# guanjq/targetdiff

Measured on AMD Instinct MI355X. Metric: ligands/sec (1000-step sampling, 100 samples/pocket) at 1/2/4/8 MI355X, higher is better.
Workload: dtype f32

## Files before the change

targetdiff_amd/csrc/node.hip:

```cpp

#include <type_traits>
#include "td_device.h"
#include "td_internal.h"

constexpr int NP_CHUNK_STEPS = 16;
constexpr int NP_CHUNK_F4 = NP_CHUNK_STEPS * 64;
constexpr int NP_CHUNKS = TD_KSTEPS / NP_CHUNK_STEPS;
constexpr int NP_TSTRIDE = 36;
constexpr size_t NP_LDS_BYTES = (size_t)(2 * NP_CHUNK_F4 * 4 + 4 * 32 * NP_TSTRIDE) * sizeof(float);

__device__ __forceinline__ void gemm128_lds(const float4 (&a)[16], const float4 *__restrict__ B,
                                            const float4 *__restrict__ next, float4 *__restrict__ bufs, int &cur,
                                            int tid, int lane, floatx16 (&acc)[4]) {
#pragma unroll
    for (int ch = 0; ch < NP_CHUNKS; ++ch) {
        const float4 *src = ch + 1 < NP_CHUNKS ? B + (size_t)(ch + 1) * NP_CHUNK_F4 : next;
        if (src) {
            float4 *dst = bufs + (cur ^ 1) * NP_CHUNK_F4 + (tid & ~63);
            const int nthr = blockDim.x;
            for (int u = 0; u < NP_CHUNK_F4; u += nthr) td_glds16(src + u + tid, dst + u);
        }
        const float4 *bl = bufs + cur * NP_CHUNK_F4 + lane;
#pragma unroll
        for (int s = 0; s < NP_CHUNK_STEPS; ++s) {
// ... 100 lines not shown
        int seen = 0;
        unsigned sel = 0;
        for (int b = 0; b < 5; ++b)
            if ((mat_mask >> b) & 1u) {
                if (seen == unit) sel = 1u << b;
                ++seen;
            }
        mat_mask = sel;
    }
    constexpr size_t MAT_F4 = (size_t)TD_KSTEPS * 64;
    const float4 *Bp = reinterpret_cast<const float4 *>(st.projB);
    const float4 *seq[6];
    int mats[6], nseq = 0;
    for (int mat = 0; mat < 5; ++mat)
        if ((mat_mask >> mat) & 1u) { seq[nseq] = Bp + (size_t)mat * MAT_F4; mats[nseq++] = mat; }
    if ((mat_mask >> 4) & 1u) { seq[nseq] = reinterpret_cast<const float4 *>(st.q3B); mats[nseq++] = 5; }
    for (int u = tid; u < NP_CHUNK_F4; u += blockDim.x) bufs[u] = seq[0][u];
    __syncthreads();
    int cur = 0;
    floatx16 acc[4];
    for (int si = 0; si < nseq; ++si) {
        const int mat = mats[si];
        const float *bias = mat < 5 ? st.projBias + mat * TD_H : st.q3Bias;
#pragma unroll
        for (int t = 0; t < 4; ++t) {
            const float bv = bias[32 * t + c];
#pragma unroll
            for (int r = 0; r < 16; ++r) acc[t][r] = bv;
        }
        const float4 *next = si + 1 < nseq ? seq[si + 1] : nullptr;
        gemm128_lds(a, seq[si], next, bufs, cur, tid, lane, acc);
        if (mat < 4) {
#pragma unroll
            for (int r = 0; r < 16; ++r) {
                const int orow = out_row(r);
                if (orow >= 0) {
#pragma unroll
                    for (int t = 0; t < 4; ++t) P[(size_t)orow * (4 * TD_H) + mat * TD_H + 32 * t + c] = acc[t][r];
                }
            }
        } else if (mat == 4) {
            float gam[4], bet[4];
#pragma unroll
            for (int t = 0; t < 4; ++t) {
                gam[t] = st.qGamma[32 * t + c];
                bet[t] = st.qBeta[32 * t + c];
            }
#pragma unroll
            for (int r = 0; r < 16; ++r) {
                const float s1 = (acc[0][r] + acc[1][r]) + (acc[2][r] + acc[3][r]);
                const float mean = td_sum32(s1) * (1.0f / TD_H);
                const float d0 = acc[0][r] - mean, d1 = acc[1][r] - mean, d2 = acc[2][r] - mean, d3 = acc[3][r] - mean;
                const float var = td_sum32((d0 * d0 + d1 * d1) + (d2 * d2 + d3 * d3)) * (1.0f / TD_H);
                const float rstd = __frsqrt_rn(var + 1e-5f);
                acc[0][r] = fmaxf(d0 * rstd * gam[0] + bet[0], 0.f);
                acc[1][r] = fmaxf(d1 * rstd * gam[1] + bet[1], 0.f);
                acc[2][r] = fmaxf(d2 * rstd * gam[2] + bet[2], 0.f);
                acc[3][r] = fmaxf(d3 * rstd * gam[3] + bet[3], 0.f);
            }
#pragma unroll
            for (int t = 0; t < 4; ++t) {
#pragma unroll
                for (int r = 0; r < 16; ++r) tb[td_erow(r, hi) * NP_TSTRIDE + c] = acc[t][r];
#pragma unroll
                for (int mm = 0; mm < 4; ++mm)
                    a[4 * t + mm] = *reinterpret_cast<const float4 *>(tb + c * NP_TSTRIDE + 8 * mm + 4 * hi);
            }
        } else {
#pragma unroll
            for (int r = 0; r < 16; ++r) {
                const int orow = out_row(r);
                if (orow >= 0) {
#pragma unroll
                    for (int t = 0; t < 4; ++t) q[(size_t)orow * TD_H + 32 * t + c] = acc[t][r];
                }
            }
        }
    }
}

__device__ __forceinline__ void td_glds16_asm_s(const uint4 *gsrc_base, uint32_t lane_bytes, uint32_t lds_wave_base) {
    asm volatile("s_mov_b32 m0, %2\n\ts_nop 0\n\tglobal_load_lds_dwordx4 %0, %1" : : "v"(lane_bytes), "s"(gsrc_base), "s"(lds_wave_base) : "memory", "m0");
}
template <bool ASYNC, bool BPIPE>
__global__ __launch_bounds__(256, 2) void node_proj_split_kernel(NpArgs args, const float *__restrict__ h) {
    int bx = blockIdx.x, si = 0;
    while (si + 1 < args.nseg && bx >= args.seg[si].blocks) { bx -= args.seg[si].blocks; ++si; }
    const NpSeg &sg = args.seg[si];
    const TdNodeStage st = sg.st;
    const int32_t *__restrict__ rows = sg.rows;
    float *__restrict__ P = sg.P, *__restrict__ q = sg.q;
    unsigned mat_mask = sg.mask;
    int64_t N = sg.N;
    int unit = -1;
    if (sg.units > 1) {
        unit = bx % sg.units;
        bx /= sg.units;
    }
    if (sg.count_ptr) {
        N = *sg.count_ptr;
        if ((int64_t)bx * (blockDim.x >> 1) >= N) return;
    }
    extern __shared__ __attribute__((aligned(16))) float lds[];
    uint4 *bufs = reinterpret_cast<uint4 *>(lds);
    const int tid = threadIdx.x, lane = tid & 63, wave = tid >> 6;
    float *tb = lds + 2 * NPS_CHUNK_U4 * 4 + wave * 32 * NP_TSTRIDE;
    const int c = lane & 31, hi = lane >> 5;
    const int64_t row0 = ((int64_t)bx * (blockDim.x >> 6) + wave) * 32;
    if (unit >= 0) {
        int seen = 0;
        unsigned sel = 0;
        for (int b = 0; b < 5; ++b)
            if ((mat_mask >> b) & 1u) {
                if (seen == unit) sel = 1u << b;
                ++seen;
            }
        mat_mask = sel;
    }
    const unsigned seq_mask = (mat_mask & 0x1fu) | (((mat_mask >> 4) & 1u) << 5);
    if (!seq_mask) return;
    constexpr size_t MAT_U4 = (size_t)NPS_CHUNKS * NPS_CHUNK_U4;
    const uint4 *Bp = reinterpret_cast<const uint4 *>(st.projB3), *Bq3 = reinterpret_cast<const uint4 *>(st.q3B3);
    auto mat_after = [&](int m) -> int {
        const unsigned rest = seq_mask & ~((2u << m) - 1u);
        return rest ? __builtin_ctz(rest) : -1;
    };
    auto mat_ptr = [&](int m) -> const uint4 * { return m < 5 ? Bp + (size_t)m * MAT_U4 : Bq3; };
    int mat = __builtin_ctz(seq_mask);
    float *sbias = lds + 2 * NPS_CHUNK_U4 * 4 + 4 * 32 * NP_TSTRIDE;
    {
        const uint4 *first = mat_ptr(mat);
        for (int u = tid; u < NPS_CHUNK_U4; u += blockDim.x) bufs[u] = first[u];
        for (int u = tid; u < NPS_BIAS_FLOATS; u += blockDim.x) sbias[u] = u < 5 * TD_H ? st.projBias[u] : st.q3Bias[u - 5 * TD_H];
    }
    uint4 ap[3][8];
    int orow4[4];
    {
        const int64_t aslot = row0 + c;
        const int64_t arow = aslot < N ? (rows ? (int64_t)rows[aslot] : aslot) : -1;
#pragma unroll
        for (int k = 0; k < 4; ++k) orow4[k] = __shfl((int)arow, (lane >> 3) + 8 * k);
        float4 a[16];
#pragma unroll
        for (int m = 0; m < 16; ++m)
            a[m] = (arow >= 0) ? *reinterpret_cast<const float4 *>(h + arow * TD_H + 8 * m + 4 * hi) : make_float4(0.f, 0.f, 0.f, 0.f);
        td_split_tile(a, ap);
    }
    __syncthreads();
    int cur = 0;
    const int64_t row0s = ((int64_t)bx * (blockDim.x >> 6) + __builtin_amdgcn_readfirstlane(wave)) * 32;
    const bool direct = !rows && row0s + 32 <= N;
    floatx16 keep[2];
    for (; mat >= 0; mat = mat_after(mat)) {
        const float *bias = sbias + mat * TD_H;
        const uint4 *B = mat_ptr(mat);
        const int mat_next = mat_after(mat);
#pragma unroll
        for (int half = 0; half < 2; ++half) {
            floatx16 acc[2];
#pragma unroll
            for (int t = 0; t < 2; ++t) {
                const float bv = bias[64 * half + 32 * t + c];
#pragma unroll
                for (int r = 0; r < 16; ++r) acc[t][r] = bv;
            }
#pragma unroll
            for (int kc = 0; kc < 2; ++kc) {
                const int chunk = 2 * half + kc;
                const uint4 *src = chunk + 1 < NPS_CHUNKS ? B + (size_t)(chunk + 1) * NPS_CHUNK_U4
                                                            : (mat_next >= 0 ? mat_ptr(mat_next) : nullptr);
                if constexpr (ASYNC) {
                    if (src) {
                        const uint32_t lbase = __builtin_amdgcn_readfirstlane(
                            (uint32_t)(uintptr_t)(__attribute__((address_space(3))) void *)(bufs + (cur ^ 1) * NPS_CHUNK_U4 + (tid & ~63)));
#pragma unroll
                        for (int u = 0; u < NPS_CHUNK_U4 / 256; ++u) {
                            td_glds16_asm_s(src + u * 256, (uint32_t)tid * 16u, lbase + u * 256 * 16);
                        }
                    }
                } else if (src) {
                    uint4 *dst = bufs + (cur ^ 1) * NPS_CHUNK_U4 + (tid & ~63);
                    for (int u = 0; u < NPS_CHUNK_U4; u += 256)
                        td_glds16(reinterpret_cast<const float4 *>(src + u + tid), reinterpret_cast<float4 *>(dst + u));
                }
                const uint4 *bl = bufs + cur * NPS_CHUNK_U4 + lane;
                uint4 b[2][3][2];
                auto load_b = [&](int ss, uint4 (&bb)[3][2]) {
#pragma unroll
                    for (int p = 0; p < 3; ++p)
#pragma unroll
                        for (int t = 0; t < 2; ++t) bb[p][t] = bl[((ss * 3 + p) * 2 + t) * 64];
                };
                if constexpr (BPIPE) load_b(0, b[0]);
#pragma unroll
                for (int ss = 0; ss < 4; ++ss) {
                    const int s = 4 * kc + ss;
                    uint4 (&bc)[3][2] = b[BPIPE ? (ss & 1) : 0];
                    if constexpr (BPIPE) {
                        if (ss + 1 < 4) load_b(ss + 1, b[(ss + 1) & 1]);
                        __builtin_amdgcn_sched_barrier(0);
                    } else
                        load_b(ss, bc);
#pragma unroll
                    for (int t = 0; t < 2; ++t) acc[t] = td_mfma_bf16(ap[1][s], bc[1][t], acc[t]);
#pragma unroll
                    for (int t = 0; t < 2; ++t) acc[t] = td_mfma_bf16(ap[2][s], bc[0][t], acc[t]);
#pragma unroll
                    for (int t = 0; t < 2; ++t) acc[t] = td_mfma_bf16(ap[0][s], bc[2][t], acc[t]);
#pragma unroll
                    for (int t = 0; t < 2; ++t) acc[t] = td_mfma_bf16(ap[1][s], bc[0][t], acc[t]);
#pragma unroll
                    for (int t = 0; t < 2; ++t) acc[t] = td_mfma_bf16(ap[0][s], bc[1][t], acc[t]);
#pragma unroll
                    for (int t = 0; t < 2; ++t) acc[t] = td_mfma_bf16(ap[0][s], bc[0][t], acc[t]);
                    if constexpr (BPIPE) __builtin_amdgcn_sched_barrier(0);
                }
                if constexpr (ASYNC) asm volatile("s_waitcnt vmcnt(0)" : : : "memory");
                __syncthreads();
                cur ^= 1;
            }
            if (mat != 4) {
                float *out = mat < 4 ? P + mat * TD_H + 64 * half : q + 64 * half;
                const size_t ld = mat < 4 ? (size_t)(4 * TD_H) : (size_t)TD_H;
                if (direct) {
                    auto store_tiles = [&](float *base, auto ldc) {
                        constexpr int LD = (int)decltype(ldc)::value;
                        const __amdgpu_buffer_rsrc_t rs = __builtin_amdgcn_make_buffer_rsrc(base + (size_t)row0s * LD, 0, 32 * LD * 4, 0x00020000);
                        const int voff = ((4 * hi) * LD + c) * 4;
#pragma unroll
                        for (int t = 0; t < 2; ++t)
#pragma unroll
                            for (int r = 0; r < 16; ++r)
                                __builtin_amdgcn_raw_buffer_store_b32(__float_as_uint(acc[t][r]), rs, voff, (td_erow(r, 0) * LD + 32 * t) * 4, 0);
                    };
                    if (mat < 4) store_tiles(out, std::integral_constant<int, 4 * TD_H>());
                    else store_tiles(out, std::integral_constant<int, TD_H>());
                } else
#pragma unroll
                for (int t = 0; t < 2; ++t) {
#pragma unroll
                    for (int r = 0; r < 16; ++r) tb[td_erow(r, hi) * NP_TSTRIDE + c] = acc[t][r];
#pragma unroll
                    for (int k = 0; k < 4; ++k) {
                        const float4 v = *reinterpret_cast<const float4 *>(tb + ((lane >> 3) + 8 * k) * NP_TSTRIDE + 4 * (lane & 7));
                        if (orow4[k] >= 0) *reinterpret_cast<float4 *>(out + (size_t)orow4[k] * ld + 32 * t + 4 * (lane & 7)) = v;
                    }
                }
            } else if (half == 0) {
                keep[0] = acc[0];
                keep[1] = acc[1];
            } else {
                float gam[4], bet[4];
#pragma unroll
                for (int t = 0; t < 4; ++t) {
                    gam[t] = st.qGamma[32 * t + c];
                    bet[t] = st.qBeta[32 * t + c];
                }
#pragma unroll
                for (int r = 0; r < 16; ++r) {
                    const float s1 = (keep[0][r] + keep[1][r]) + (acc[0][r] + acc[1][r]);
                    const float mean = td_sum32(s1) * (1.0f / TD_H);
                    const float d0 = keep[0][r] - mean, d1 = keep[1][r] - mean, d2 = acc[0][r] - mean, d3 = acc[1][r] - mean;
                    const float var = td_sum32((d0 * d0 + d1 * d1) + (d2 * d2 + d3 * d3)) * (1.0f / TD_H);
                    const float rstd = __frsqrt_rn(var + 1e-5f);
                    keep[0][r] = fmaxf(d0 * rstd * gam[0] + bet[0], 0.f);
                    keep[1][r] = fmaxf(d1 * rstd * gam[1] + bet[1], 0.f);
                    acc[0][r] = fmaxf(d2 * rstd * gam[2] + bet[2], 0.f);
                    acc[1][r] = fmaxf(d3 * rstd * gam[3] + bet[3], 0.f);
                }
                float4 a[16];
#pragma unroll
                for (int t = 0; t < 4; ++t) {
#pragma unroll
                    for (int r = 0; r < 16; ++r)
                        tb[td_erow(r, hi) * NP_TSTRIDE + c] = t == 0 ? keep[0][r] : t == 1 ? keep[1][r] : t == 2 ? acc[0][r] : acc[1][r];
#pragma unroll
                    for (int mm = 0; mm < 4; ++mm)
                        a[4 * t + mm] = *reinterpret_cast<const float4 *>(tb + c * NP_TSTRIDE + 8 * mm + 4 * hi);
                }
                td_split_tile(a, ap);
            }
        }
    }
}

static int np_fill(NpSeg &g, const TdNodeStage &st, const int32_t *rows, const int32_t *count_ptr, int64_t N, unsigned mask,
                   float *P, float *q, bool split_units, int rows_per_wg) {
    g.st = st; g.rows = rows; g.count_ptr = count_ptr; g.N = N; g.P = P; g.q = q; g.mask = mask;
    g.units = split_units ? __builtin_popcount(mask & 0x1fu) : 1;
    g.blocks = (int)((N + rows_per_wg - 1) / rows_per_wg) * g.units;
    return g.blocks;
}

static int np_launch(const NpArgs &a, const float *h, unsigned total_blocks, hipStream_t s) {
    bool split = true;
    for (int i = 0; i < a.nseg; ++i) split = split && a.seg[i].st.use_split && a.seg[i].st.projB3 != nullptr;
    const dim3 grid(total_blocks), block(256);
    if (split && a.seg[0].st.async_copy && a.seg[0].st.bpipe) return td_launch<node_proj_split_kernel<true, true>>(grid, block, NPS_LDS_BYTES, s, a, h);
    if (split && a.seg[0].st.async_copy) return td_launch<node_proj_split_kernel<true, false>>(grid, block, NPS_LDS_BYTES, s, a, h);
    if (split) return td_launch<node_proj_split_kernel<false, false>>(grid, block, NPS_LDS_BYTES, s, a, h);
    return td_launch<node_proj_kernel>(grid, block, NP_LDS_BYTES, s, a, h);
}

int td_launch_node_proj(const TdNodeStage &st, const float *h, int64_t N, const int32_t *rows, unsigned mat_mask,
                        float *P, float *q, hipStream_t s, const int32_t *count_ptr, const int32_t *rows2, int64_t N2,
                        unsigned mask2) {
    if (N == 0 || mat_mask == 0) return TD_OK;
    if (!rows2 || N2 == 0 || (mask2 & 0x1fu) == 0) { rows2 = nullptr; N2 = 0; mask2 = 0; }
    NpArgs a;
    a.nseg = 0;
    unsigned total = 0;
    total += np_fill(a.seg[a.nseg++], st, rows, count_ptr, N, mat_mask, P, q, N <= TD_SMALL_BATCH_ROWS, 128);
    if (rows2) total += np_fill(a.seg[a.nseg++], st, rows2, nullptr, N2, mask2, P, q, true, 128);
    return np_launch(a, h, total, s);
}

int td_launch_node_proj_pair(const TdNodeStage &hx, const int32_t *hop_rows, const int32_t *hop_count,
                             const int32_t *lig_rows, int64_t Nl, float *Px, float *qx, const TdNodeStage &nx,
                             const int32_t *rows, const int32_t *count_ptr, float *P, float *q, const float *h, int64_t N,
                             hipStream_t s) {
    if (N == 0) return TD_OK;
    NpArgs a;
    a.nseg = 0;
    unsigned total = 0;
    const bool one_round = (N + 127) / 128 <= 512;
    total += np_fill(a.seg[a.nseg++], nx, rows, rows ? count_ptr : nullptr, N, 0x1f, P, q, N <= TD_SMALL_BATCH_ROWS, 128);
    if (Nl > 0) total += np_fill(a.seg[a.nseg++], hx, lig_rows, nullptr, Nl, 0x15, Px, qx, true, 128);
    total += np_fill(a.seg[a.nseg++], hx, hop_rows, hop_rows ? hop_count : nullptr, N, 0x0a, Px, qx, one_round, 128);
    return np_launch(a, h, total, s);
}

template <bool LN>
__global__ __launch_bounds__(256, 2) void egnn_node_kernel(const float4 *__restrict__ B, const float *__restrict__ b1,
                                                           const float *__restrict__ b2, const float *__restrict__ mi,
                                                           float *__restrict__ h, int64_t N, const float *__restrict__ gamma,
                                                           const float *__restrict__ beta) {
    extern __shared__ __attribute__((aligned(16))) float lds[];
    float4 *bufs = reinterpret_cast<float4 *>(lds);
    const int tid = threadIdx.x, lane = tid & 63, wave = tid >> 6;
    float *tb = lds + 2 * NP_CHUNK_F4 * 4 + wave * 32 * NP_TSTRIDE;
    const int c = lane & 31, hi = lane >> 5;
    const int64_t row0 = ((int64_t)blockIdx.x * 4 + wave) * 32;
    const int64_t arow = row0 + c < N ? row0 + c : -1;
    const float4 *B0 = B, *B1 = B + (size_t)TD_KSTEPS * 64, *B2 = B + (size_t)2 * TD_KSTEPS * 64;
    for (int u = tid; u < NP_CHUNK_F4; u += blockDim.x) bufs[u] = B0[u];
    __syncthreads();
    int cur = 0;
    float4 a[16];
    floatx16 acc[4];
#pragma unroll
    for (int t = 0; t < 4; ++t) {
        const float bv = b1[32 * t + c];
#pragma unroll
        for (int r = 0; r < 16; ++r) acc[t][r] = bv;
    }
#pragma unroll
    for (int m = 0; m < 16; ++m)
        a[m] = arow >= 0 ? *reinterpret_cast<const float4 *>(mi + arow * TD_H + 8 * m + 4 * hi) : make_float4(0.f, 0.f, 0.f, 0.f);
    gemm128_lds(a, B0, B1, bufs, cur, tid, lane, acc);
#pragma unroll
    for (int m = 0; m < 16; ++m)
        a[m] = arow >= 0 ? *reinterpret_cast<const float4 *>(h + arow * TD_H + 8 * m + 4 * hi) : make_float4(0.f, 0.f, 0.f, 0.f);
    gemm128_lds(a, B1, B2, bufs, cur, tid, lane, acc);
    if constexpr (LN) {
        float gam[4], bet[4];
#pragma unroll
        for (int t = 0; t < 4; ++t) { gam[t] = gamma[32 * t + c]; bet[t] = beta[32 * t + c]; }
#pragma unroll
        for (int r = 0; r < 16; ++r) {
            const float mean = td_sum32((acc[0][r] + acc[1][r]) + (acc[2][r] + acc[3][r])) * (1.0f / TD_H);
            const float d0 = acc[0][r] - mean, d1 = acc[1][r] - mean, d2 = acc[2][r] - mean, d3 = acc[3][r] - mean;
            const float rstd = __frsqrt_rn(td_sum32((d0 * d0 + d1 * d1) + (d2 * d2 + d3 * d3)) * (1.0f / TD_H) + 1e-5f);
            acc[0][r] = fmaxf(d0 * rstd * gam[0] + bet[0], 0.f);
            acc[1][r] = fmaxf(d1 * rstd * gam[1] + bet[1], 0.f);
            acc[2][r] = fmaxf(d2 * rstd * gam[2] + bet[2], 0.f);
            acc[3][r] = fmaxf(d3 * rstd * gam[3] + bet[3], 0.f);
        }
    }
#pragma unroll
    for (int t = 0; t < 4; ++t) {
#pragma unroll
// ... 37 lines not shown
```

targetdiff_amd/csrc/pack.cpp:

```cpp
#include <algorithm>
#include <atomic>
#include <cmath>
#include <cstdarg>
#include <cstdio>
#include <cstdlib>
#include <cstring>
#include <mutex>
#include <new>
#include <vector>

#include "td_device.h"
#include "td_internal.h"
#include "td_api.h"

using namespace tdapi;

namespace tdapi {



struct FoldedMlp {
    std::vector<float> w0, b0, g, b, w3, b3v;
    const float *b3;
    float ln_c1 = 1.f / 128.f, ln_c2 = 1e-5f;
// ... 277 lines not shown
            for (int r = 0; r < 4; ++r)
                for (int lane = 0; lane < 64; ++lane)
                    q16[((size_t)hb * 4 + r) * 64 + lane] = m.w3[(size_t)(lane & 15) * TD_H + 16 * hb + 4 * (lane >> 4) + r];
    }
    if (alt == 1) {
        o.Walt = pk.alloc((size_t)4 * 16 * 2 * 2 * 16 * 4);
        float *q = pk.data.data() + o.Walt;
        for (int t = 0; t < 4; ++t)
            for (int r = 0; r < 16; ++r)
                for (int jq = 0; jq < 2; ++jq)
                    for (int hi = 0; hi < 2; ++hi)
                        for (int c = 0; c < 16; ++c)
                            for (int jj = 0; jj < 4; ++jj) {
                                const int n = 32 * t + (r & 3) + 8 * (r >> 2) + 4 * hi;
                                q[((((((size_t)t * 16 + r) * 2 + jq) * 2 + hi) * 16 + c) * 4) + jj] =
                                    m.w3[(size_t)(8 * c + 4 * jq + jj) * TD_H + n];
                            }
        o.Walt16 = pk.alloc((size_t)8 * 4 * 2 * 64 * 4);
        float *q16 = pk.data.data() + o.Walt16;
        for (int hb = 0; hb < 8; ++hb)
            for (int r = 0; r < 4; ++r)
                for (int jq = 0; jq < 2; ++jq)
                    for (int lane = 0; lane < 64; ++lane)
                        for (int jj = 0; jj < 4; ++jj) {
                            const int head = lane & 15, k = 16 * hb + 4 * (lane >> 4) + r;
                            q16[(((((size_t)hb * 4 + r) * 2 + jq) * 64 + lane) * 4) + jj] =
                                m.w3[(size_t)(8 * head + 4 * jq + jj) * TD_H + k];
                        }
    } else if (alt == 2) {
        o.Walt = pk.alloc((size_t)32 * TD_H * 4);
        float *q = pk.data.data() + o.Walt;
        for (int d = 0; d < 8; ++d)
            for (int kq = 0; kq < 32; ++kq)
                for (int head = 0; head < TD_HEADS; ++head)
                    for (int kk = 0; kk < 4; ++kk)
                        q[((((size_t)d * 32 + kq) * TD_HEADS + head) * 4) + kk] = m.w3[(size_t)(8 * head + d) * TD_H + 4 * kq + kk];
    }
    return o;
}

struct NodeOff { size_t projB, projBias, qGamma, qBeta, q3B, q3Bias, projB3, q3B3; };

NodeOff pack_node_stage(Packer &pk, const MlpSrc &k, const MlpSrc &v, const MlpSrc &q, int in_dim) {
    NodeOff o;
    const int hi_col = in_dim - 2 * TD_H, hj_col = in_dim - TD_H;
    o.projB = pack_B128(pk, k.w0, in_dim, hi_col);
    pack_B128(pk, k.w0, in_dim, hj_col);
    pack_B128(pk, v.w0, in_dim, hi_col);
    pack_B128(pk, v.w0, in_dim, hj_col);
    pack_B128(pk, q.w0, TD_H, 0);
    o.projBias = pk.alloc(5 * TD_H);
    memcpy(pk.data.data() + o.projBias + 0 * TD_H, k.b0, TD_H * sizeof(float));
    memcpy(pk.data.data() + o.projBias + 2 * TD_H, v.b0, TD_H * sizeof(float));
    memcpy(pk.data.data() + o.projBias + 4 * TD_H, q.b0, TD_H * sizeof(float));
    o.qGamma = pack_vec(pk, q.g, TD_H);
    o.qBeta = pack_vec(pk, q.b, TD_H);
    o.q3B = pack_B128(pk, q.w3, TD_H, 0);
    o.q3Bias = pack_vec(pk, q.b3, TD_H);
    o.projB3 = pack_B128_split(pk, k.w0, in_dim, hi_col);
    pack_B128_split(pk, k.w0, in_dim, hj_col);
    pack_B128_split(pk, v.w0, in_dim, hi_col);
    pack_B128_split(pk, v.w0, in_dim, hj_col);
    pack_B128_split(pk, q.w0, TD_H, 0);
    o.q3B3 = pack_B128_split(pk, q.w3, TD_H, 0);
    return o;
}

float gaussian_coeff(const float *off) {
    const float d = off[1] - off[0];
    return -0.5f / (d * d);
}


}

namespace {
enum OptKind { OPT_FLAG, OPT_CLAMPED, OPT_RANGED };
struct OptRow { const char *name; int TdOptions::*field; OptKind kind; int lo, hi; };
const OptRow OPTIONS[] = {
    {"h2x_fused", &TdOptions::h2x_fused, OPT_FLAG, 0, 1},
    {"node_proj_split", &TdOptions::node_proj_split, OPT_FLAG, 0, 1},
    {"node_proj_bpipe", &TdOptions::node_proj_bpipe, OPT_FLAG, 0, 1},
    {"node_proj_async", &TdOptions::node_proj_async, OPT_FLAG, 0, 1},
    {"edge_key_split", &TdOptions::edge_key_split, OPT_FLAG, 0, 1},
    {"edge_first_layer_f16", &TdOptions::edge_first_layer_f16, OPT_FLAG, 0, 1},
    {"edge_second_layer_f16", &TdOptions::edge_second_layer_f16, OPT_FLAG, 0, 1},
    {"edge_row_dealing", &TdOptions::edge_row_dealing, OPT_CLAMPED, 0, 2},
    {"session_hop_levels", &TdOptions::session_hop_levels, OPT_RANGED, 1, TD_HOP_LEVELS},
    {"session_forward_reach", &TdOptions::session_forward_reach, OPT_FLAG, 0, 1},
    {"session_step_lists", &TdOptions::session_step_lists, OPT_FLAG, 0, 1},
    {"session_share_pockets", &TdOptions::session_share_pockets, OPT_FLAG, 0, 1},
};
struct ReadOnlyRow { const char *name; int td_model::*field; };
const ReadOnlyRow READ_ONLY[] = {{"fold_dead_units", &td_model::fold_dead_units}, {"fold_fp32_mlps", &td_model::fold_fp32_mlps}};

template <class Row, size_t N>
const Row *find_row(const Row (&rows)[N], const char *name) {
    for (const Row &r : rows)
        if (strcmp(r.name, name) == 0) return &r;
    return nullptr;
}

void apply_options(td_model *m) {
    const TdOptions &o = m->opt;
    m->gate.use_split = o.edge_key_split != 0;
    for (int l = 0; l < m->cfg.num_layers * stage_rows(m->cfg); ++l) {
        TdLayer &L = m->layers[l];
        for (TdNodeStage *n : {&L.nodeX2h, &L.nodeH2x}) { n->use_split = o.node_proj_split != 0; n->bpipe = o.node_proj_bpipe != 0; n->async_copy = o.node_proj_async != 0; }
        for (TdEdgeMlp *e : {&L.hk, &L.hv, &L.xk, &L.xv}) {
            e->use_split = e->R16q && o.edge_key_split != 0;
            e->l1_f16 = e->R16h && e->f16_safe && o.edge_first_layer_f16 != 0;
            e->l2_f16 = e->f16_safe && o.edge_second_layer_f16 != 0;
            e->deal_rows = o.edge_row_dealing;
        }
    }
}
}

extern "C" size_t td_model_num_weights(const td_config *cfg) {
    if (!cfg) return 0;
    const td_config &c = *cfg;
    const int H = c.hidden_dim, E = H - 1, KV = kv_in(c);
    size_t n = (size_t)E * c.protein_feat_dim + E + (size_t)E * c.ligand_num_classes + E;
    n += c.num_r_gaussian + (c.ew_net_type == 0 ? mlp_floats(c.num_r_gaussian, H, 1) : 0);
    const size_t nx = num_x2h(c), nh = num_h2x(c);
    size_t xs = 2 * mlp_floats(KV, H, H) + mlp_floats(H, H, H), hs = mlp_floats(KV, H, H) + mlp_floats(KV, H, c.n_heads) + mlp_floats(H, H, H);
    if (c.ew_net_type == 1) { xs += 4 * c.num_r_gaussian + 1; hs += 4 * c.num_r_gaussian + 1; }
    if (c.ew_net_type == 3) xs += H + 1;
    if (c.x2h_out_fc) xs += mlp_floats(2 * H, H, H);
    n += (size_t)c.num_layers * (c.num_r_gaussian + nx * xs + nh * hs);
    n += (size_t)H * H + H + (size_t)c.ligand_num_classes * H + c.ligand_num_classes;
    return n;
}

extern "C" int td_model_create(const td_config *cfg, const float *host_weights, size_t num_weights,
                               const float *host_schedules, size_t num_schedule_floats, td_model **out) {
    if (!cfg || !host_weights || !out) { td_set_error("td_model_create: null argument"); return TD_EINVAL; }
    const td_config &c = *cfg;
    if (!config_supported(c)) {
        td_set_error("td_model_create: unsupported configuration (need hidden 128, 16 heads, 20 gaussians, edge_feat_dim 4, "
                     "knn / max_num_neighbors in 1..%d, cutoff_mode knn|hybrid|radius; got %d/%d/%d/%d, knn %d, cutoff_mode %d, "
                     "radius %g, max_num_neighbors %d)", TD_MAX_FANIN, c.hidden_dim, c.n_heads, c.num_r_gaussian,
                     c.edge_feat_dim, c.knn, c.cutoff_mode, (double)c.radius, c.max_num_neighbors);
        return TD_EINVAL;
    }
    if (num_weights != td_model_num_weights(cfg)) {
        td_set_error("td_model_create: weight blob has %zu floats, expected %zu", num_weights, td_model_num_weights(cfg));
        return TD_EINVAL;
    }
    if (host_schedules && num_schedule_floats != (size_t)7 * c.num_timesteps &&
        num_schedule_floats != (size_t)8 * c.num_timesteps && num_schedule_floats != (size_t)10 * c.num_timesteps) {
        td_set_error("td_model_create: schedule blob has %zu floats, expected %zu (sampling) or %zu (+ alphas_cumprod)",
                     num_schedule_floats, (size_t)7 * c.num_timesteps, (size_t)8 * c.num_timesteps);
        return TD_EINVAL;
    }
    const bool has_rc = host_schedules && num_schedule_floats == (size_t)10 * c.num_timesteps;
    const bool has_abar = has_rc || (host_schedules && num_schedule_floats == (size_t)8 * c.num_timesteps);
    if (c.num_blocks < 0 || c.num_blocks > 8) {
        td_set_error("td_model_create: num_blocks must be 1 .. 8 (0 = 1), got %d", c.num_blocks);
        return TD_EINVAL;
    }
    if (c.ew_net_type < 0 || c.ew_net_type > 3 || (c.x2h_out_fc != 0 && c.x2h_out_fc != 1)) {
        td_set_error("td_model_create: ew_net_type must be 0 ('global'), 1 ('r'), 2 (none) or 3 ('m'), x2h_out_fc 0 or 1; got %d / %d",
                     c.ew_net_type, c.x2h_out_fc);
        return TD_EINVAL;
    }
    if (c.num_x2h < 0 || c.num_x2h > 4 || c.num_h2x < 0 || c.num_h2x > 4) {
        td_set_error("td_model_create: num_x2h / num_h2x must be 1 .. 4 (0 = 1), got %d / %d", c.num_x2h, c.num_h2x);
        return TD_EINVAL;
    }
    if (stage_rows(c) > 1 && c.sync_twoup) {
        td_set_error("td_model_create: sync_twoup with several stages per layer is not built");
        return TD_EINVAL;
    }
    if (c.sync_twoup != 0 && c.sync_twoup != 1) { td_set_error("td_model_create: sync_twoup must be 0 or 1, got %d", c.sync_twoup); return TD_EINVAL; }
    if (c.ew_net_type != 0 && !default_graph(c)) {
        td_set_error("td_model_create: ew_net_type 'r' / 'm' / none runs on the 32-slot graphs only (knn <= 32, or radius with a cap <= 32)");
        return TD_EINVAL;
    }
    if (c.model_mean_type != 0 && c.model_mean_type != 1) {
        td_set_error("td_model_create: model_mean_type must be 0 ('C0') or 1 ('noise'), got %d", c.model_mean_type);
        return TD_EINVAL;
    }
    if (c.model_mean_type == 1 && !has_rc) {
        td_set_error("td_model_create: model_mean_type 'noise' needs the 10 schedule arrays (sqrt_recip_alphas_cumprod, sqrt_recipm1_alphas_cumprod)");
        return TD_EINVAL;
    }
    const int H = TD_H, E = H - 1, F = c.protein_feat_dim, C = c.ligand_num_classes, KV = kv_in(c), L = c.num_layers;
    Cursor cur{host_weights, num_weights};
    const float *Wp = cur.take((size_t)E * F), *bp = cur.take(E);
    const float *Wl = cur.take((size_t)E * C), *bl = cur.take(E);
// ... 201 lines not shown
```

targetdiff_amd/csrc/td_internal.h:

```cpp
#pragma once

#include <hip/hip_runtime.h>
#include <stddef.h>
#include <stdint.h>

#include <atomic>
#include <type_traits>

#include "../../include/targetdiff_hip.h"

constexpr int TD_H = 128;
constexpr int TD_HEADS = 16;
constexpr int TD_DH = 8;
constexpr int TD_K = 32;
constexpr int TD_NG = 20;
constexpr int TD_SLOTK = 24;
constexpr int TD_SLOT_STEPS = TD_SLOTK / 2;
constexpr int TD_KSTEPS = TD_H / 2;
constexpr int TD_MAXC = 16;
constexpr int TD_SMALL_BATCH_ROWS = 16384;

void td_set_error(const char *fmt, ...);
#define TD_CHECK_HIP(expr)                                                                       \
    do {                                                                                         \
        hipError_t _e = (expr);                                                                  \
        if (_e != hipSuccess) {                                                                  \
            td_set_error("%s failed: %s (%s:%d)", #expr, hipGetErrorString(_e), __FILE__, __LINE__); \
            return TD_EHIP;                                                                      \
        }                                                                                        \
    } while (0)

struct TdLdsOnce {
    std::atomic<unsigned long long> mask{0};
};
inline int td_set_lds(TdLdsOnce &once, const void *fn, size_t bytes) {
    int dev = 0;
    TD_CHECK_HIP(hipGetDevice(&dev));
    const unsigned long long bit = 1ull << (dev & 63);
    if (once.mask.load(std::memory_order_acquire) & bit) return TD_OK;
    TD_CHECK_HIP(hipFuncSetAttribute(fn, hipFuncAttributeMaxDynamicSharedMemorySize, (int)bytes));
    once.mask.fetch_or(bit, std::memory_order_release);
    return TD_OK;
}
template <auto Kernel, class... Args>
int td_launch(dim3 grid, dim3 block, size_t lds_bytes, hipStream_t s, const Args &...args) {
    static TdLdsOnce once;
    const int rc = td_set_lds(once, reinterpret_cast<const void *>(Kernel), lds_bytes);
    if (rc != TD_OK) return rc;
    Kernel<<<grid, block, lds_bytes, s>>>(args...);
    TD_CHECK_HIP(hipGetLastError());
    return TD_OK;
}

struct TdEdgeMlp {
    const float *R;
    const float *gamma;
    const float *beta;
    const float *W2;
    const float *b2;
    const float *R16;
    const float *Walt16;
    const float *Walt;
    const float *R16q;
    const float *R16h;
    float ln_c1, ln_c2;
    float w2_bound;
    bool l2_f16;
    bool l1_f16;
    bool z_plain;
    bool use_split;
    int deal_rows;
    bool f16_safe;
};

struct TdNodeStage {
    const float *projB;
    const float *projBias;
    const float *qGamma, *qBeta;
    const float *q3B;
    const float *q3Bias;
    const float *projB3;
    const float *q3B3;
    bool use_split;
    bool bpipe;
    bool async_copy;
};

struct TdNodeOut {
    const float *B;
    const float *b1, *gamma, *beta, *b2;
};

struct TdLayer {
    TdNodeStage nodeX2h, nodeH2x;
    TdEdgeMlp hk, hv, xk, xv;
    const float *ew_x2h, *ew_h2x;
    const float *gate_m;
    TdNodeOut nodeOut;
    const float *offsets;
    float coeff;
};

struct TdGate {
    const float *R;
    const float *b0, *gamma, *beta, *w3;
    float b3;
    const float *offsets;
    float coeff;
    const float *R16q;
    float ln_c1, ln_c2;
    bool use_split;
};

struct TdEmbed {
    const float *WpT;
    const float *bp;
    const float *WlT;
    const float *bl;
};

struct TdHead {
    const float *W0T;
    const float *b0;
    const float *W2T;
    const float *b2;
};

struct TdEgnnLayer {
    TdNodeStage proj;
    const float *W2f;
    const float *Wxf;
    const float *vec;
    const float *nodeB;
    const float *nb1, *nb2;
};

constexpr int TD_PROP_H = 256;
constexpr int TD_PROP_G = 64;
constexpr int TD_PROP_ACT_NONE = 0, TD_PROP_ACT_RELU = 1, TD_PROP_ACT_SSP = 2;
constexpr int TD_PROP_EPI_NONE = 0, TD_PROP_EPI_RELU_MASK = 1, TD_PROP_EPI_SSP_DERIV = 2;
constexpr int TD_PROP_XTY_CHUNKS = 64;
struct TdPropLayer {
    const float *projW, *projB;
    const float *W1f;
    const float *W2f;
    const float *b2, *winf, *binf;
    const float *offset;
    const float *n1W, *n1b, *n2W, *n2b;
};

struct TdSchedules {
    const float *c0, *ct, *logvar, *log_a, *log_1ma, *log_ca, *log_1mca;
    const float *abar;
    const float *rc, *rm1;
};

struct TdOptions {
    int h2x_fused = 1;
    int node_proj_split = 1;
    int edge_key_split = 1;
    int edge_first_layer_f16 = 1;
    int edge_second_layer_f16 = 1;
    int session_hop_levels = 4;
    int session_forward_reach = 1;
    int edge_row_dealing = 2;
    int node_proj_bpipe = 0;
    int node_proj_async = 1;
    int session_share_pockets = 1;
    int session_step_lists = 1;
};

struct td_model {
    td_config cfg;
    TdOptions opt;
    float *blob;
    size_t blob_floats;
    TdEmbed emb;
    TdGate gate;
    TdLayer *layers;
    TdHead head;
    TdSchedules sched;
    unsigned option_epoch = 0;
    int fold_dead_units = 0;
    int fold_fp32_mlps = 0;
};

int td_launch_graph_ptr(const int64_t *batch, int64_t N, int64_t B, int32_t *ptr, hipStream_t s);
int td_launch_node_gid(const int32_t *node_ptr, int64_t N, int64_t B, int32_t *gid, hipStream_t s);
int td_launch_pack_x(const float *x3, const uint8_t *mask, int64_t N, float4 *x4, hipStream_t s);
int td_launch_unpack_x(const float4 *x4, int64_t N, float *x3, hipStream_t s);
int td_launch_knn(const float4 *x4, const int32_t *node_ptr, const int32_t *gid, int64_t N, int max_graph_nodes,
                  int32_t *nbr, hipStream_t s, int k = TD_K);
int td_launch_compose(const td_model *m, const float *ppos, const float *pv, const int32_t *pptr, int64_t Np,
                      const float *lpos, const int64_t *lv, const int32_t *lptr, int64_t Nl, int64_t B,
                      float *h, float4 *x4, int32_t *node_ptr, int32_t *gid, int32_t *lig_node, int32_t *prot_node,
                      hipStream_t s, const float *gbias = nullptr);
int td_launch_knn_rows(const float4 *x4, const int32_t *node_ptr, const int32_t *gid, const int32_t *rows, int64_t count,
                       int max_graph_nodes, int32_t *nbr, hipStream_t s, int k = TD_K);
int td_launch_knn_static(const float4 *x4, const int32_t *node_ptr, const int32_t *gid, const int32_t *rows, int64_t count,
                         int max_graph_nodes, int32_t *nbr, unsigned long long *skeys, hipStream_t s, int k = TD_K);
int td_launch_knn_merge(const float4 *x4, const int32_t *node_ptr, const int32_t *pptr, const int32_t *gid,
                        const int32_t *prot_rows, int64_t Np, const unsigned long long *skeys, const int32_t *snbr,
                        const float *h0, const float *h1s, const float *ews, int32_t *nbr, float *h, float *ew,
                        uint8_t *clean, uint8_t *flags2, hipStream_t s, int k = TD_K, const int32_t *lig_rows = nullptr, int64_t Nl = 0,
                        int max_graph_nodes = 0, const int32_t *cgraph = nullptr, const int32_t *cbase = nullptr);
int td_launch_pocket_hash(const float *ppos, const float *pv, const int32_t *pptr, int64_t B, int F, unsigned long long *out, hipStream_t s);
int td_launch_pocket_verify(const float *ppos, const float *pv, const int32_t *pptr, int64_t B, int F, const int32_t *cand, int32_t *flags,
                            hipStream_t s);
int td_launch_compact_rows(const void *src, const int32_t *rows, int64_t n_rows, int row_bytes, void *dst, hipStream_t s);
int td_launch_compact_dirty(const uint8_t *clean, const float4 *x4, int64_t N, int32_t *rows, int32_t *count,
                            hipStream_t s);
int td_launch_forward_reach(const uint8_t *clean, const float4 *x4, const int32_t *nbr, int64_t N, uint8_t *flags2,
                            int32_t *rows_on, int32_t *rows_off, int32_t *counts2, uint8_t *clean_to_zero, hipStream_t s);
int td_launch_restore_rows(const int32_t *rows, const int32_t *count_ptr, int64_t max_rows, const float *hs, float *h,
                           hipStream_t s, const int32_t *gid = nullptr, const int32_t *node_ptr = nullptr, const int32_t *cbase = nullptr);
constexpr int TD_HOP_LEVELS = 4;
int td_launch_hop_levels(const int32_t *lig_node, int64_t Nl, const int32_t *nbr, int64_t N, uint8_t *flags,
                         int32_t *rows, int32_t *counts, int levels, hipStream_t s, bool zeroed = false);
int td_launch_gate16(const TdGate &g, const float4 *x4, const int32_t *nbr, int64_t N, const int32_t *rows,
                     const int32_t *count_ptr, float *ew, hipStream_t s, const int32_t *chunk_node);
struct TdStepLists {
    int32_t *dirty_rows, *dirty_count;
    int32_t *reach_rows, *rest_rows, *reach_counts;
    int32_t *level_rows, *level_counts;
    int levels;
    int32_t *dirty_chunks = nullptr, *dirty_chunk_count = nullptr;
};
int td_launch_step_lists(const uint8_t *clean, const float4 *x4, const int32_t *nbr, const int32_t *node_ptr, int64_t N,
                         int64_t B, int max_nodes, const TdStepLists &out, hipStream_t s, const int32_t *cptr = nullptr,
                         const int32_t *chunk_node = nullptr);
struct TdStepReset {
    int32_t *c0 = nullptr, *c1 = nullptr, *c2 = nullptr;
    int n0 = 0, n1 = 0, n2 = 0;
    uint8_t *flags2 = nullptr;
};
int td_launch_ligand_update(const td_model *m, const float *lpos, const int64_t *lv, const int32_t *lig_node, int64_t Nl,
                            float *h, float4 *x4, hipStream_t s, const TdStepReset *reset = nullptr, const float *gbias = nullptr,
                            const int32_t *gid = nullptr);
int td_launch_ligand_list(const uint8_t *mask, int64_t N, int32_t *lig_node, int32_t *count, hipStream_t s);
int td_launch_node_proj(const TdNodeStage &st, const float *h, int64_t N, const int32_t *rows, unsigned mat_mask,
                        float *P, float *q, hipStream_t s, const int32_t *count_ptr = nullptr,
                        const int32_t *rows2 = nullptr, int64_t N2 = 0, unsigned mask2 = 0);
int td_launch_node_proj_pair(const TdNodeStage &hx, const int32_t *hop_rows, const int32_t *hop_count,
                             const int32_t *lig_rows, int64_t Nl, float *Px, float *qx, const TdNodeStage &nx,
                             const int32_t *rows, const int32_t *count_ptr, float *P, float *q, const float *h, int64_t N,
                             hipStream_t s);
int td_launch_node_output(const TdNodeOut &no, const float *out, float *h, int64_t N, hipStream_t s);
int td_launch_layer_gate(const float *w, const float *offsets, float coeff, const float4 *x4, const int32_t *nbr, int64_t N, float *ew,
                         hipStream_t s);
int td_launch_gate(const TdGate &g, const float4 *x4, const int32_t *nbr, int64_t N, const int32_t *rows,
// ... 311 lines not shown
```

Measured before the change: 27.94.

## Stream node projection weights through a four-slot async LDS ring

Adds a ring-buffered variant of the split node-projection kernel. Weight matrices are cut into half-chunk stages and held in a four-slot LDS ring filled with global_load_lds. Copies are interleaved between MFMA steps, and barriers wait on partial vmcnt counts, so each wave waits only for the stage it needs rather than a whole chunk. The option is on by default. It adds hand-written waitcnt and barrier logic, and a wrong count would be a correctness risk.

After: 27.85. No clear change (-0.3%).

```diff
diff --git a/targetdiff_amd/csrc/node.hip b/targetdiff_amd/csrc/node.hip
--- a/targetdiff_amd/csrc/node.hip
+++ b/targetdiff_amd/csrc/node.hip
@@ -206,8 +206,18 @@
 __device__ __forceinline__ void td_glds16_asm_s(const uint4 *gsrc_base, uint32_t lane_bytes, uint32_t lds_wave_base) {
     asm volatile("s_mov_b32 m0, %2\n\ts_nop 0\n\tglobal_load_lds_dwordx4 %0, %1" : : "v"(lane_bytes), "s"(gsrc_base), "s"(lds_wave_base) : "memory", "m0");
 }
-template <bool ASYNC, bool BPIPE>
+constexpr int NPS_STAGE_U4 = NPS_CHUNK_U4 / 2;
+constexpr int NPS_STAGES = 8;
+constexpr int NPS_RING = 4;
+constexpr int NPS_STAGE_COPIES = NPS_STAGE_U4 / 256;
+template <int N>
+__device__ __forceinline__ void td_ring_barrier() {
+    asm volatile("s_waitcnt vmcnt(%0) lgkmcnt(0)\n\ts_barrier" : : "n"(N) : "memory");
+}
+template <bool ASYNC, bool BPIPE, bool RING = false>
 __global__ __launch_bounds__(256, 2) void node_proj_split_kernel(NpArgs args, const float *__restrict__ h) {
+    static_assert(!RING || (ASYNC && !BPIPE), "the ring is a form of the async copy");
+    static_assert(NPS_STAGES % NPS_RING == 0, "a matrix starts at slot 0");
     int bx = blockIdx.x, si = 0;
     while (si + 1 < args.nseg && bx >= args.seg[si].blocks) { bx -= args.seg[si].blocks; ++si; }
     const NpSeg &sg = args.seg[si];
@@ -254,7 +264,12 @@
     float *sbias = lds + 2 * NPS_CHUNK_U4 * 4 + 4 * 32 * NP_TSTRIDE;
     {
         const uint4 *first = mat_ptr(mat);
-        for (int u = tid; u < NPS_CHUNK_U4; u += blockDim.x) bufs[u] = first[u];
+        if constexpr (RING) {
+            const uint32_t lbase = __builtin_amdgcn_readfirstlane((uint32_t)(uintptr_t)(__attribute__((address_space(3))) void *)(bufs + (tid & ~63)));
+#pragma unroll
+            for (int u = 0; u < (NPS_RING - 1) * NPS_STAGE_COPIES; ++u) td_glds16_asm_s(first + u * 256, (uint32_t)tid * 16u, lbase + u * 256 * 16);
+        } else
+            for (int u = tid; u < NPS_CHUNK_U4; u += blockDim.x) bufs[u] = first[u];
         for (int u = tid; u < NPS_BIAS_FLOATS; u += blockDim.x) sbias[u] = u < 5 * TD_H ? st.projBias[u] : st.q3Bias[u - 5 * TD_H];
     }
     uint4 ap[3][8];
@@ -270,7 +285,8 @@
             a[m] = (arow >= 0) ? *reinterpret_cast<const float4 *>(h + arow * TD_H + 8 * m + 4 * hi) : make_float4(0.f, 0.f, 0.f, 0.f);
         td_split_tile(a, ap);
     }
-    __syncthreads();
+    if constexpr (RING) td_ring_barrier<0>();
+    else __syncthreads();
     int cur = 0;
     const int64_t row0s = ((int64_t)bx * (blockDim.x >> 6) + __builtin_amdgcn_readfirstlane(wave)) * 32;
     const bool direct = !rows && row0s + 32 <= N;
@@ -290,6 +306,48 @@
             }
 #pragma unroll
             for (int kc = 0; kc < 2; ++kc) {
+                if constexpr (RING) {
+#pragma unroll
+                    for (int rr = 0; rr < 2; ++rr) {
+                        const int r = 4 * half + 2 * kc + rr;
+                        const int fr = r + NPS_RING - 1;
+                        const uint4 *src = fr < NPS_STAGES ? B + (size_t)fr * NPS_STAGE_U4
+                                                           : (mat_next >= 0 ? mat_ptr(mat_next) + (size_t)(fr - NPS_STAGES) * NPS_STAGE_U4 : nullptr);
+                        const uint32_t lbase = __builtin_amdgcn_readfirstlane(
+                            (uint32_t)(uintptr_t)(__attribute__((address_space(3))) void *)(bufs + (fr % NPS_RING) * NPS_STAGE_U4 + (tid & ~63)));
+                        const uint4 *bl = bufs + (r % NPS_RING) * NPS_STAGE_U4 + lane;
+                        int u = 0;
+#pragma unroll
+                        for (int ss = 0; ss < 2; ++ss) {
+                            const int s = 2 * (r & 3) + ss;
+                            uint4 bc[3][2];
+#pragma unroll
+                            for (int p = 0; p < 3; ++p)
+#pragma unroll
+                                for (int t = 0; t < 2; ++t) bc[p][t] = bl[((ss * 3 + p) * 2 + t) * 64];
+                            constexpr int PA[6] = {1, 2, 0, 1, 0, 0}, PB[6] = {1, 0, 2, 0, 1, 0};
+#pragma unroll
+                            for (int i = 0; i < 6; ++i) {
+#pragma unroll
+                                for (int t = 0; t < 2; ++t) acc[t] = td_mfma_bf16(ap[PA[i]][s], bc[PB[i]][t], acc[t]);
+                                if ((i == 1 || (i == 3 && ss == 0)) && src) {
+                                    __builtin_amdgcn_sched_barrier(0);
+                                    td_glds16_asm_s(src + u * 256, (uint32_t)tid * 16u, lbase + u * 256 * 16);
+                                    __builtin_amdgcn_sched_barrier(0);
+                                    ++u;
+                                }
+                            }
+                        }
+                        static_assert(NPS_STAGE_COPIES == 3, "two copies behind the first k-step, one behind the second");
+                        const bool last = mat_next < 0;
+                        if (last && r == NPS_STAGES - 1) break;
+                        const int behind = !last || r + 3 < NPS_STAGES ? 2 : NPS_STAGES - 2 - r;
+                        if (behind == 2) td_ring_barrier<2 * NPS_STAGE_COPIES>();
+                        else if (behind == 1) td_ring_barrier<NPS_STAGE_COPIES>();
+                        else td_ring_barrier<0>();
+                    }
+                    continue;
+                }
                 const int chunk = 2 * half + kc;
                 const uint4 *src = chunk + 1 < NPS_CHUNKS ? B + (size_t)(chunk + 1) * NPS_CHUNK_U4
                                                             : (mat_next >= 0 ? mat_ptr(mat_next) : nullptr);
@@ -421,6 +479,7 @@
     for (int i = 0; i < a.nseg; ++i) split = split && a.seg[i].st.use_split && a.seg[i].st.projB3 != nullptr;
     const dim3 grid(total_blocks), block(256);
     if (split && a.seg[0].st.async_copy && a.seg[0].st.bpipe) return td_launch<node_proj_split_kernel<true, true>>(grid, block, NPS_LDS_BYTES, s, a, h);
+    if (split && a.seg[0].st.async_copy && a.seg[0].st.ring) return td_launch<node_proj_split_kernel<true, false, true>>(grid, block, NPS_LDS_BYTES, s, a, h);
     if (split && a.seg[0].st.async_copy) return td_launch<node_proj_split_kernel<true, false>>(grid, block, NPS_LDS_BYTES, s, a, h);
     if (split) return td_launch<node_proj_split_kernel<false, false>>(grid, block, NPS_LDS_BYTES, s, a, h);
     return td_launch<node_proj_kernel>(grid, block, NP_LDS_BYTES, s, a, h);
diff --git a/targetdiff_amd/csrc/pack.cpp b/targetdiff_amd/csrc/pack.cpp
--- a/targetdiff_amd/csrc/pack.cpp
+++ b/targetdiff_amd/csrc/pack.cpp
@@ -383,6 +383,7 @@
     {"node_proj_split", &TdOptions::node_proj_split, OPT_FLAG, 0, 1},
     {"node_proj_bpipe", &TdOptions::node_proj_bpipe, OPT_FLAG, 0, 1},
     {"node_proj_async", &TdOptions::node_proj_async, OPT_FLAG, 0, 1},
+    {"node_proj_ring", &TdOptions::node_proj_ring, OPT_FLAG, 0, 1},
     {"edge_key_split", &TdOptions::edge_key_split, OPT_FLAG, 0, 1},
     {"edge_first_layer_f16", &TdOptions::edge_first_layer_f16, OPT_FLAG, 0, 1},
     {"edge_second_layer_f16", &TdOptions::edge_second_layer_f16, OPT_FLAG, 0, 1},
@@ -407,7 +408,7 @@
     m->gate.use_split = o.edge_key_split != 0;
     for (int l = 0; l < m->cfg.num_layers * stage_rows(m->cfg); ++l) {
         TdLayer &L = m->layers[l];
-        for (TdNodeStage *n : {&L.nodeX2h, &L.nodeH2x}) { n->use_split = o.node_proj_split != 0; n->bpipe = o.node_proj_bpipe != 0; n->async_copy = o.node_proj_async != 0; }
+        for (TdNodeStage *n : {&L.nodeX2h, &L.nodeH2x}) { n->use_split = o.node_proj_split != 0; n->bpipe = o.node_proj_bpipe != 0; n->async_copy = o.node_proj_async != 0; n->ring = o.node_proj_ring != 0; }
         for (TdEdgeMlp *e : {&L.hk, &L.hv, &L.xk, &L.xv}) {
             e->use_split = e->R16q && o.edge_key_split != 0;
             e->l1_f16 = e->R16h && e->f16_safe && o.edge_first_layer_f16 != 0;
diff --git a/targetdiff_amd/csrc/td_internal.h b/targetdiff_amd/csrc/td_internal.h
--- a/targetdiff_amd/csrc/td_internal.h
+++ b/targetdiff_amd/csrc/td_internal.h
@@ -84,6 +84,7 @@
     bool use_split;
     bool bpipe;
     bool async_copy;
+    bool ring;
 };
 
 struct TdNodeOut {
@@ -166,6 +167,7 @@
     int edge_row_dealing = 2;
     int node_proj_bpipe = 0;
     int node_proj_async = 1;
+    int node_proj_ring = 1;
     int session_share_pockets = 1;
     int session_step_lists = 1;
 };
```
